# tinganchen/AlignQ

Measured on AMD Instinct MI355X. Metric: images/sec (train step, CDF+ADMM) ResNet-20 8-bit, higher is better.
Workload: dtype f32; 1 GPU; resnet20 CIFAR-shape 3x32x32, 8W/8A CDF+ADMM full train step (cdf_alignment_admm/resnet-20-cifar-10), batch 128/GPU, HIP-graph replay, batch-norm folded into the site kernels, channels-last tensors, all Conv2d_Q convolutions on alignq_conv*_nhwc (exact-product bf16 MFMA); global_batch=128, parallelism=dp1

## Files before the change

alignq_amd/csrc/conv_kernels.hip:

```cpp
#include <hip/hip_runtime.h>
#include <stdint.h>
#include <stdlib.h>

#include "../../include/alignq.h"
#include "site_internal.h"
#include "store_forms.h"
#include "wgrad_reduce_body.h"

namespace {

using namespace alignq_wgr;

typedef __bf16 bf16x8 __attribute__((ext_vector_type(8)));
typedef __bf16 bf16x4 __attribute__((ext_vector_type(4)));
typedef float f32x4 __attribute__((ext_vector_type(4)));
typedef short s16x4 __attribute__((ext_vector_type(4)));

#ifdef ALIGNQ_STAMPS
__device__ unsigned long long g_conv_stamps[64];
__device__ unsigned long long g_conv_blk[2][4096];
#define STAMP(on, i)                                                          \
  do {                                                                        \
    if ((on) && threadIdx.x == 0) g_conv_stamps[i] = wall_clock64();          \
  } while (0)
#define BSTAMP(which)                                                                          \
  do {                                                                                         \
    if (threadIdx.x == 0 && blockIdx.x < 4096) g_conv_blk[which][blockIdx.x] = wall_clock64(); \
  } while (0)
#else
#define STAMP(on, i) do { } while (0)
#define BSTAMP(which) do { } while (0)
#endif

__device__ __forceinline__ s16x4 tr_read(const __bf16* p) {
  return __builtin_amdgcn_ds_read_tr16_b64_v4i16((__attribute__((address_space(3))) s16x4*)(p));
}
__device__ __forceinline__ bf16x8 join8(s16x4 a, s16x4 b) {
  typedef short s16x8 __attribute__((ext_vector_type(8)));
  s16x8 v = {a[0], a[1], a[2], a[3], b[0], b[1], b[2], b[3]};
  return __builtin_bit_cast(bf16x8, v);
}


template <int xb>
__device__ __forceinline__ f32x4 fetch_act4(const float* __restrict__ x, int64_t off) {
  if constexpr (xb == 0) return *reinterpret_cast<const f32x4*>(x + off);
  if constexpr (xb == 2) {
    const s16x4 b = *reinterpret_cast<const s16x4*>(reinterpret_cast<const short*>(x) + off);
    return (f32x4){(float)b[0], (float)b[1], (float)b[2], (float)b[3]};
  }
  const char4 b = *reinterpret_cast<const char4*>(reinterpret_cast<const signed char*>(x) + off);
  return (f32x4){(float)b.x, (float)b.y, (float)b.z, (float)b.w};
}

struct BnLazy {
  const float* z;
  const float* ab;
  const float* save;
  const float* ktot;
  const float* part = nullptr;
  int n_tiles = 0, tile_f = 0;
  double inv_n = 1.0;
  float* dgamma = nullptr;
  float* dbeta = nullptr;
};

template <int C>
__device__ __forceinline__ void bn_totals_lds(const BnLazy& t, float* __restrict__ kt, bool publish) {
  static_assert(256 % C == 0, "thread -> (channel, group)");
  __shared__ double red[256][2];
  constexpr int G = 256 / C;
  const int tid = threadIdx.x;
  const int cp = C < t.tile_f ? C : t.tile_f;
  const int cyc = C / cp, cnt = t.n_tiles / cyc;
  const int c = tid % C, grp = tid / C;
  const int e = c % cp, t_first = c / cp;
  double s0 = 0, s1 = 0;
  constexpr int U = 16;
  for (int i0 = grp; i0 < cnt; i0 += G * U) {
    float2 v[U];
#pragma unroll
    for (int u = 0; u < U; u++) {
      const int i = i0 + u * G;
      const int ic = i < cnt ? i : cnt - 1;
      v[u] = *reinterpret_cast<const float2*>(t.part + ((int64_t)(ic * cyc + t_first) * cp + e) * 2);
    }
#pragma unroll
    for (int u = 0; u < U; u++) {
      if (i0 + u * G < cnt) { s0 += v[u].x; s1 += v[u].y; }
    }
  }
  red[tid][0] = s0;
  red[tid][1] = s1;
  __syncthreads();
  if (tid < C) {
    double t0 = 0, t1 = 0;
#pragma unroll
    for (int g = 0; g < G; g++) { t0 += red[g * C + tid][0]; t1 += red[g * C + tid][1]; }
    kt[tid] = (float)(t0 * t.inv_n);
    kt[C + tid] = (float)(t1 * t.inv_n);
    if (publish) {
      if (t.dbeta) t.dbeta[tid] = (float)t0;
      if (t.dgamma) t.dgamma[tid] = (float)t1;
    }
  }
  __syncthreads();
}

__device__ __forceinline__ float4 bn_lazy4(const float4& g, const float4& z, const float4& a, const float4& m, const float4& is,
                                           const float4& k0, const float4& k1) {
  float4 o;
  o.x = a.x * (g.x - k0.x - (z.x - m.x) * is.x * k1.x);
  o.y = a.y * (g.y - k0.y - (z.y - m.y) * is.y * k1.y);
  o.z = a.z * (g.z - k0.z - (z.z - m.z) * is.z * k1.z);
  o.w = a.w * (g.w - k0.w - (z.w - m.w) * is.w * k1.w);
  return o;
}

template <int C> constexpr int conv_cp() { return C == 16 ? 16 : (C == 32 ? 48 : C + 8); }
template <int C, int WD, int PT>
struct ConvLds {
  static constexpr int kBf16 = 3 * ((PT / WD) + 2) * (WD + 2) * conv_cp<C>();
};

template <int C, int WD, int PT, bool DGRAD, int XB = 0, bool IMG = false>
__device__ __forceinline__ void conv3x3_body(const float* __restrict__ x, const float* __restrict__ w,
                                             float* __restrict__ y, int H, int total_rows, float nlev, __bf16* lds,
                                             int block, const float* __restrict__ add,
                                             float* __restrict__ bn_part = nullptr, int n_wg = 0,
                                             BnLazy lazy = BnLazy{nullptr, nullptr, nullptr, nullptr}, float xlev = 1.0f) {
  static_assert(XB == 0 || !DGRAD, "the data gradient reads fp32 dy");
  constexpr int xb = XB;
  constexpr int TR = PT / WD;
  constexpr int NS = (9 * C + 31) / 32;
  constexpr int NCG = C / 16;
  constexpr int NPP = 4 / NCG;
  constexpr int NG = PT / 16;
  constexpr int LW = WD + 2;
  constexpr int CP = conv_cp<C>();
  constexpr int LROWS = TR + 2;
  constexpr int ARR = LROWS * LW * CP;
  static_assert(3 * ARR == ConvLds<C, WD, PT>::kBf16, "LDS size");
  __bf16* Xhi = lds;
  __bf16* Xmi = lds + ARR;
  __bf16* Xlo = lds + 2 * ARR;

  const int tid = threadIdx.x, lane = tid & 63, wv = tid >> 6;
  const int row0 = block * TR;
  const int img_lo = (row0 / H) * H, img_hi = img_lo + H;
  [[maybe_unused]] constexpr int SB = DGRAD ? 8 : 0;
  STAMP(block == 0, SB + 0);
  const int cog = wv % NCG, pp = wv / NCG;
  const int m = lane & 15, q = lane >> 4;
  bf16x8 ab[NS];
  {
    constexpr int C4 = C / 4;
    constexpr int N4 = LROWS * LW * C4;
    constexpr int NIT = (N4 + 255) / 256;
    float4 v[NIT];
#pragma unroll
    for (int it = 0; it < NIT; it++) {
      const int i = tid + 256 * it;
      const int c4 = i % C4, col = (i / C4) % LW, lr = i / (C4 * LW);
      const int grow = row0 + lr - 1;
      const bool ok = i < N4 && col >= 1 && col <= WD && grow >= img_lo && grow < img_hi && grow < total_rows;
      const int64_t off = ok ? ((int64_t)grow * WD + (col - 1)) * C + 4 * c4 : 0;
      const f32x4 ld = fetch_act4<XB>(x, off);
      v[it] = ok ? make_float4(ld[0], ld[1], ld[2], ld[3]) : make_float4(0.f, 0.f, 0.f, 0.f);
    }
    STAMP(block == 0, SB + 1);
    if (DGRAD && lazy.z) {
      float4 zz[NIT];
#pragma unroll
      for (int it = 0; it < NIT; it++) {
        const int i = tid + 256 * it;
        const int c4 = i % C4, col = (i / C4) % LW, lr = i / (C4 * LW);
        const int grow = row0 + lr - 1;
        const bool ok = i < N4 && col >= 1 && col <= WD && grow >= img_lo && grow < img_hi && grow < total_rows;
        zz[it] = *reinterpret_cast<const float4*>(lazy.z + (ok ? ((int64_t)grow * WD + (col - 1)) * C + 4 * c4 : 0));
      }
      const int c4t = tid % C4;
      const float4 a4 = *reinterpret_cast<const float4*>(lazy.ab + 4 * c4t);
      const float4 m4 = *reinterpret_cast<const float4*>(lazy.save + 4 * c4t);
      const float4 i4 = *reinterpret_cast<const float4*>(lazy.save + C + 4 * c4t);
      float4 k0, k1;
      if (lazy.part) {
        __shared__ __attribute__((aligned(16))) float kt[2 * C];
        bn_totals_lds<C>(lazy, kt, block == 0);
        k0 = *reinterpret_cast<const float4*>(kt + 4 * c4t);
        k1 = *reinterpret_cast<const float4*>(kt + C + 4 * c4t);
      } else {
        k0 = *reinterpret_cast<const float4*>(lazy.ktot + 4 * c4t);
        k1 = *reinterpret_cast<const float4*>(lazy.ktot + C + 4 * c4t);
      }
#pragma unroll
      for (int it = 0; it < NIT; it++) {
        const int i = tid + 256 * it;
        const int col = (i / C4) % LW, lr = i / (C4 * LW);
        const int grow = row0 + lr - 1;
        const bool ok = i < N4 && col >= 1 && col <= WD && grow >= img_lo && grow < img_hi && grow < total_rows;
        if (ok) v[it] = bn_lazy4(v[it], zz[it], a4, m4, i4, k0, k1);
      }
    }
#pragma unroll
    for (int it = 0; it < NIT; it++) {
      const int i = tid + 256 * it;
      if (i < N4) {
        const int c4 = i % C4, col = (i / C4) % LW, lr = i / (C4 * LW);
        bf16x4 h4, m4, l4;
        const float vv[4] = {v[it].x, v[it].y, v[it].z, v[it].w};
#pragma unroll
        for (int e = 0; e < 4; e++) {
          const __bf16 hi = (__bf16)vv[e];
          const float r1 = vv[e] - (float)hi;
          const __bf16 mi = (__bf16)r1;
          const float r2 = r1 - (float)mi;
          h4[e] = hi; m4[e] = mi; l4[e] = (__bf16)r2;
        }
        const int o = (lr * LW + col) * CP + 4 * c4;
        *reinterpret_cast<bf16x4*>(Xhi + o) = h4;
        *reinterpret_cast<bf16x4*>(Xmi + o) = m4;
        *reinterpret_cast<bf16x4*>(Xlo + o) = l4;
      }
    }
    STAMP(block == 0, SB + 2);
    if constexpr (IMG) {
      const bf16x8* __restrict__ wi = reinterpret_cast<const bf16x8*>(w) + (cog * NS) * 64 + lane;
#pragma unroll
      for (int s = 0; s < NS; s++) ab[s] = wi[s * 64];
    } else {
#pragma unroll
      for (int s = 0; s < NS; s++) {
        const int k0 = 32 * s + 8 * q;
        const bool live = k0 / C < 9;
        const int tap = live ? k0 / C : 8, c0 = k0 % C;
        float wr[8];
        if (!DGRAD) {
          const float* p = w + ((int64_t)(cog * 16 + m) * 9 + tap) * C + c0;
          const float4 a4 = *reinterpret_cast<const float4*>(p), b4 = *reinterpret_cast<const float4*>(p + 4);
          wr[0] = a4.x; wr[1] = a4.y; wr[2] = a4.z; wr[3] = a4.w; wr[4] = b4.x; wr[5] = b4.y; wr[6] = b4.z; wr[7] = b4.w;
        } else {
#pragma unroll
          for (int j = 0; j < 8; j++) wr[j] = w[((int64_t)(c0 + j) * 9 + (8 - tap)) * C + cog * 16 + m];
        }
#pragma unroll
        for (int j = 0; j < 8; j++) ab[s][j] = (__bf16)rintf((live ? wr[j] : 0.f) * nlev);
      }
    }
    STAMP(block == 0, SB + 3);
  }
  __syncthreads();
  constexpr int GW = NG / NPP;
  static_assert(NG % NPP == 0, "every wave takes the same number of pixel groups");
  int bo[GW];
  f32x4 acc[GW];
#pragma unroll
  for (int gi = 0; gi < GW; gi++) {
    const int p = (pp + gi * NPP) * 16 + (lane & 15);
    bo[gi] = ((p / WD) * LW + (p % WD)) * CP;
    acc[gi] = (f32x4){0.f, 0.f, 0.f, 0.f};
  }
  constexpr int GB = (DGRAD && GW > 2) ? 2 : GW;
  static_assert(GW % GB == 0, "whole batches of groups");
#pragma unroll
  for (int g0 = 0; g0 < GW; g0 += GB) {
    bf16x8 bh[2][GB], bm[2][GB], bl[2][GB];
#pragma unroll
    for (int s = 0; s <= NS; s++) {
      if (s < NS) {
        const int k0 = 32 * s + 8 * q;
        const bool live = k0 / C < 9;
        const int tap = live ? k0 / C : 8, c0 = k0 % C;
        const int to = ((tap / 3) * LW + (tap % 3)) * CP + c0;
#pragma unroll
        for (int gi = 0; gi < GB; gi++) {
          const int o = bo[g0 + gi] + to;
          bh[s & 1][gi] = *reinterpret_cast<const bf16x8*>(Xhi + o);
          bm[s & 1][gi] = *reinterpret_cast<const bf16x8*>(Xmi + o);
          if (DGRAD || xb == 0) bl[s & 1][gi] = *reinterpret_cast<const bf16x8*>(Xlo + o);
          if ((9 * C) % 32 != 0 && !live) {
#pragma unroll
            for (int j = 0; j < 8; j++) { bh[s & 1][gi][j] = (__bf16)0.f; bm[s & 1][gi][j] = (__bf16)0.f; bl[s & 1][gi][j] = (__bf16)0.f; }
          }
        }
      }
      __builtin_amdgcn_sched_barrier(0);
      if (s > 0) {
        const int u = s - 1;
#pragma unroll
        for (int gi = 0; gi < GB; gi++) {
          f32x4 a = acc[g0 + gi];
          if (DGRAD || xb == 0) a = __builtin_amdgcn_mfma_f32_16x16x32_bf16(ab[u], bl[u & 1][gi], a, 0, 0, 0);
          a = __builtin_amdgcn_mfma_f32_16x16x32_bf16(ab[u], bm[u & 1][gi], a, 0, 0, 0);
          acc[g0 + gi] = __builtin_amdgcn_mfma_f32_16x16x32_bf16(ab[u], bh[u & 1][gi], a, 0, 0, 0);
        }
      }
    }
  }
  float bs[4] = {0.f, 0.f, 0.f, 0.f}, bq[4] = {0.f, 0.f, 0.f, 0.f};
#pragma unroll
  for (int gi = 0; gi < GW; gi++) {
    const int p = (pp + gi * NPP) * 16 + (lane & 15);
    const int r = p / WD, c = p % WD;
    const int grow = row0 + r;
    if (grow < total_rows) {
      const int64_t o = ((int64_t)grow * WD + c) * C + cog * 16 + 4 * q;
      const float den = (!DGRAD && xb != 0) ? nlev * xlev : nlev;
      float4 v = make_float4(acc[gi][0] / den, acc[gi][1] / den, acc[gi][2] / den, acc[gi][3] / den);
      if (add) {
        const float4 r = *reinterpret_cast<const float4*>(add + o);
        v.x += r.x; v.y += r.y; v.z += r.z; v.w += r.w;
      }
      alignq_store::st16<alignq_store::kConvOut>(y + o, v);
      bs[0] += v.x; bs[1] += v.y; bs[2] += v.z; bs[3] += v.w;
      bq[0] += v.x * v.x; bq[1] += v.y * v.y; bq[2] += v.z * v.z; bq[3] += v.w * v.w;
    }
  }
  STAMP(block == 0, SB + 4);
  if (!DGRAD && bn_part) {
    float* red = reinterpret_cast<float*>(lds);
#define ROW_SHR_ADD(V, CTRL) V += __builtin_bit_cast(float, __builtin_amdgcn_update_dpp(0, __builtin_bit_cast(int, V), CTRL, 0xf, 0xf, false))
#pragma unroll
    for (int e = 0; e < 4; e++) {
      ROW_SHR_ADD(bs[e], 0x111); ROW_SHR_ADD(bs[e], 0x112); ROW_SHR_ADD(bs[e], 0x114); ROW_SHR_ADD(bs[e], 0x118);
      ROW_SHR_ADD(bq[e], 0x111); ROW_SHR_ADD(bq[e], 0x112); ROW_SHR_ADD(bq[e], 0x114); ROW_SHR_ADD(bq[e], 0x118);
    }
#undef ROW_SHR_ADD
    __syncthreads();
    if ((lane & 15) == 15) {
#pragma unroll
      for (int e = 0; e < 4; e++) {
        red[(wv * 16 + 4 * q + e) * 2] = bs[e];
        red[(wv * 16 + 4 * q + e) * 2 + 1] = bq[e];
      }
    }
    __syncthreads();
    if (tid < C) {
      const int cg = tid / 16, cl = tid % 16;
      float s0 = 0.f, s1 = 0.f;
#pragma unroll
      for (int ppi = 0; ppi < NPP; ppi++) {
        const int w2 = ppi * NCG + cg;
        s0 += red[(w2 * 16 + cl) * 2];
// ... 390 lines not shown
      float4 out = make_float4(acc[0] / nlev, acc[1] / nlev, acc[2] / nlev, acc[3] / nlev);
      if (add) {
        const float4 a4 = *reinterpret_cast<const float4*>(add + o);
        out.x += a4.x; out.y += a4.y; out.z += a4.z; out.w += a4.w;
      }
      alignq_store::st16<alignq_store::kConvOut>(dx + o, out);
    }
  }
}

template <int CIN, int COUT, int WDI, int KS, int PT, bool WITH1>
struct DgradS2Lds {
  static constexpr int P = KS == 3 ? 1 : 0, TR = PT / WDI;
  static constexpr int kBf16 = 3 * (((TR / 2 + P) * (WDI / 2 + P) + 1) + (WITH1 ? (TR / 2) * (WDI / 2) : 0)) * (COUT + 8);
};

template <int CIN, int COUT, int WDI, int KS, int PT, bool IMG = false>
__global__ __launch_bounds__(256) void dgrad_s2_kernel(const float* __restrict__ dy, const float* __restrict__ w,
                                                       float* __restrict__ dx, int H, int total_rows, float nlev,
                                                       const float* __restrict__ add, BnLazy lazy) {
  __shared__ __attribute__((aligned(16))) __bf16 lds[DgradS2Lds<CIN, COUT, WDI, KS, PT, false>::kBf16];
  dgrad_s2_body<CIN, COUT, WDI, KS, PT, false, IMG>(dy, w, dx, H, total_rows, nlev, add, lazy, lds, blockIdx.x);
}

template <int CIN, int COUT, int WDI, int KS, int PT>
int launch_dgrad_s2(const float* dy, const float* w, float* dx, int B, int H, float nlev, const float* add, BnLazy lazy,
                    hipStream_t st, bool img = false) {
  constexpr int TR = PT / WDI;
  static_assert(TR % 2 == 0, "even number of input rows per tile");
  if (H % TR) return ALIGNQ_EUNSUPPORTED;
  const int total_rows = B * H;
  if (img)
    hipLaunchKernelGGL((dgrad_s2_kernel<CIN, COUT, WDI, KS, PT, true>), total_rows / TR, 256, 0, st, dy, w, dx, H, total_rows, nlev,
                       add, lazy);
  else
    hipLaunchKernelGGL((dgrad_s2_kernel<CIN, COUT, WDI, KS, PT>), total_rows / TR, 256, 0, st, dy, w, dx, H, total_rows, nlev,
                       add, lazy);
  hipError_t e = hipGetLastError();
  return e == hipSuccess ? 0 : (int)e;
}

constexpr int kStemPT = 128;
__device__ __forceinline__ void stem_stage(const float* __restrict__ x, int H, int row0, __bf16* Chi, __bf16* Cmi, __bf16* Clo) {
  const int tid = threadIdx.x;
  const int pix = tid >> 1, half = tid & 1;
  const int r = pix / 32, c = pix % 32;
  const int grow = row0 + r;
  const int ih = grow % H;
  float v[16];
#pragma unroll
  for (int j = 0; j < 16; j++) {
    const int k = 16 * half + j;
    const int tap = k / 3, ci = k % 3;
    const int ky = tap / 3, kx = tap % 3;
    const int yy = ih + ky - 1, xx = c + kx - 1;
    const bool ok = k < 27 && yy >= 0 && yy < H && xx >= 0 && xx < 32;
    v[j] = x[ok ? ((int64_t)(grow + ky - 1) * 32 + xx) * 3 + ci : 0];
    if (!ok) v[j] = 0.f;
  }
  bf16x8 h[2], m[2], l[2];
#pragma unroll
  for (int j = 0; j < 16; j++) {
    const __bf16 hi = (__bf16)v[j];
    const float r1 = v[j] - (float)hi;
    const __bf16 mi = (__bf16)r1;
    h[j >> 3][j & 7] = hi; m[j >> 3][j & 7] = mi; l[j >> 3][j & 7] = (__bf16)(r1 - (float)mi);
  }
  const int o = pix * 32 + 16 * half;
  *reinterpret_cast<bf16x8*>(Chi + o) = h[0]; *reinterpret_cast<bf16x8*>(Chi + o + 8) = h[1];
  *reinterpret_cast<bf16x8*>(Cmi + o) = m[0]; *reinterpret_cast<bf16x8*>(Cmi + o + 8) = m[1];
  *reinterpret_cast<bf16x8*>(Clo + o) = l[0]; *reinterpret_cast<bf16x8*>(Clo + o + 8) = l[1];
}

__global__ __launch_bounds__(256) void stem_fwd_kernel(const float* __restrict__ x, const float* __restrict__ w,
                                                       float* __restrict__ y, int H, int total_rows, float nlev,
                                                       float* __restrict__ bn_part) {
  __shared__ __attribute__((aligned(16))) __bf16 lds[3 * kStemPT * 32];
  __bf16* Chi = lds;
  __bf16* Cmi = lds + kStemPT * 32;
  __bf16* Clo = lds + 2 * kStemPT * 32;
  const int tid = threadIdx.x, lane = tid & 63, wv = tid >> 6;
  const int row0 = blockIdx.x * 4;
  stem_stage(x, H, row0, Chi, Cmi, Clo);
  const int m = lane & 15, q = lane >> 4;
  bf16x8 ab;
#pragma unroll
  for (int j = 0; j < 8; j++) {
    const int k = 8 * q + j;
    ab[j] = (__bf16)rintf((k < 27 ? w[m * 27 + k] : 0.f) * nlev);
  }
  __syncthreads();
  float bs[4] = {0.f, 0.f, 0.f, 0.f}, bq[4] = {0.f, 0.f, 0.f, 0.f};
  for (int g = wv; g < kStemPT / 16; g += 4) {
    const int p = g * 16 + (lane & 15);
    const int o = p * 32 + 8 * q;
    f32x4 acc = {0.f, 0.f, 0.f, 0.f};
    acc = __builtin_amdgcn_mfma_f32_16x16x32_bf16(ab, *reinterpret_cast<const bf16x8*>(Clo + o), acc, 0, 0, 0);
    acc = __builtin_amdgcn_mfma_f32_16x16x32_bf16(ab, *reinterpret_cast<const bf16x8*>(Cmi + o), acc, 0, 0, 0);
    acc = __builtin_amdgcn_mfma_f32_16x16x32_bf16(ab, *reinterpret_cast<const bf16x8*>(Chi + o), acc, 0, 0, 0);
    const int grow = row0 + p / 32;
    if (grow < total_rows) {
      const float4 v = make_float4(acc[0] / nlev, acc[1] / nlev, acc[2] / nlev, acc[3] / nlev);
      alignq_store::st16<alignq_store::kConvOut>(y + ((int64_t)grow * 32 + p % 32) * 16 + 4 * q, v);
      bs[0] += v.x; bs[1] += v.y; bs[2] += v.z; bs[3] += v.w;
      bq[0] += v.x * v.x; bq[1] += v.y * v.y; bq[2] += v.z * v.z; bq[3] += v.w * v.w;
    }
  }
  if (bn_part) {
    float* red = reinterpret_cast<float*>(lds);
#define ROW_SHR_ADD(V, CTRL) V += __builtin_bit_cast(float, __builtin_amdgcn_update_dpp(0, __builtin_bit_cast(int, V), CTRL, 0xf, 0xf, false))
#pragma unroll
    for (int e = 0; e < 4; e++) {
      ROW_SHR_ADD(bs[e], 0x111); ROW_SHR_ADD(bs[e], 0x112); ROW_SHR_ADD(bs[e], 0x114); ROW_SHR_ADD(bs[e], 0x118);
      ROW_SHR_ADD(bq[e], 0x111); ROW_SHR_ADD(bq[e], 0x112); ROW_SHR_ADD(bq[e], 0x114); ROW_SHR_ADD(bq[e], 0x118);
    }
#undef ROW_SHR_ADD
    __syncthreads();
    if ((lane & 15) == 15) {
#pragma unroll
      for (int e = 0; e < 4; e++) {
        red[(wv * 16 + 4 * q + e) * 2] = bs[e];
        red[(wv * 16 + 4 * q + e) * 2 + 1] = bq[e];
      }
    }
    __syncthreads();
    if (tid < 16) {
      float s0 = 0.f, s1 = 0.f;
#pragma unroll
      for (int w2 = 0; w2 < 4; w2++) { s0 += red[(w2 * 16 + tid) * 2]; s1 += red[(w2 * 16 + tid) * 2 + 1]; }
      bn_part[((int64_t)tid * gridDim.x + blockIdx.x) * 2] = s0;
      bn_part[((int64_t)tid * gridDim.x + blockIdx.x) * 2 + 1] = s1;
    }
  }
}

__global__ __launch_bounds__(256) void stem_wgrad_kernel(const float* __restrict__ x, const float* __restrict__ dy,
                                                         float* __restrict__ slabs, int H, int n_tiles, BnLazy lazy) {
  __shared__ __attribute__((aligned(16))) __bf16 lds[3 * kStemPT * 32 + 3 * kStemPT * 16];
  __bf16* Ci[3] = {lds, lds + kStemPT * 32, lds + 2 * kStemPT * 32};
  __bf16* Di[3] = {lds + 3 * kStemPT * 32, lds + 3 * kStemPT * 32 + kStemPT * 16, lds + 3 * kStemPT * 32 + 2 * kStemPT * 16};
  const int tid = threadIdx.x, lane = tid & 63, wv = tid >> 6;
  const int g = lane >> 4, q = (lane & 15) >> 2, pcol = 4 * (lane & 3);
  f32x4 acc[2] = {{0.f, 0.f, 0.f, 0.f}, {0.f, 0.f, 0.f, 0.f}};
  __shared__ __attribute__((aligned(16))) float kt[32];
  if (lazy.z && lazy.part) bn_totals_lds<16>(lazy, kt, blockIdx.x == 0);
  for (int tile = blockIdx.x; tile < n_tiles; tile += gridDim.x) {
    const int row0 = tile * 4;
    f32x4 dvr[2], zvr[2];
#pragma unroll
    for (int it = 0; it < 2; it++) {
      const int i = tid + 256 * it;
      const int64_t off = ((int64_t)row0 * 32 + i / 4) * 16 + 4 * (tid % 4);
      dvr[it] = *reinterpret_cast<const f32x4*>(dy + off);
      zvr[it] = lazy.z ? *reinterpret_cast<const f32x4*>(lazy.z + off) : (f32x4){0.f, 0.f, 0.f, 0.f};
    }
    __syncthreads();
    stem_stage(x, H, row0, Ci[0], Ci[1], Ci[2]);
    {
      const int c4 = tid % 4;
      f32x4 la = {0, 0, 0, 0}, lm = la, li = la, lk0 = la, lk1 = la;
      if (lazy.z) {
        la = *reinterpret_cast<const f32x4*>(lazy.ab + 4 * c4);
        lm = *reinterpret_cast<const f32x4*>(lazy.save + 4 * c4);
        li = *reinterpret_cast<const f32x4*>(lazy.save + 16 + 4 * c4);
        const float* kp = lazy.part ? kt : lazy.ktot;
        lk0 = *reinterpret_cast<const f32x4*>(kp + 4 * c4);
        lk1 = *reinterpret_cast<const f32x4*>(kp + 16 + 4 * c4);
      }
#pragma unroll
      for (int it = 0; it < 2; it++) {
        const int i = tid + 256 * it;
        f32x4 dv = dvr[it];
        if (lazy.z) dv = la * (dv - lk0 - (zvr[it] - lm) * li * lk1);
        bf16x4 h4, m4, l4;
#pragma unroll
        for (int e = 0; e < 4; e++) {
          const __bf16 hi = (__bf16)dv[e];
          const float r1 = dv[e] - (float)hi;
          const __bf16 mi = (__bf16)r1;
          h4[e] = hi; m4[e] = mi; l4[e] = (__bf16)(r1 - (float)mi);
        }
        const int o = (i / 4) * 16 + 4 * c4;
        *reinterpret_cast<bf16x4*>(Di[0] + o) = h4;
        *reinterpret_cast<bf16x4*>(Di[1] + o) = m4;
        *reinterpret_cast<bf16x4*>(Di[2] + o) = l4;
      }
    }
    __syncthreads();
    {
      const int p0 = 32 * wv + 8 * g;
      bf16x8 a[3];
#pragma unroll
      for (int t = 0; t < 3; t++) {
        const __bf16* pa = Di[t] + (p0 + q) * 16 + pcol;
        a[t] = join8(tr_read(pa), tr_read(pa + 4 * 16));
      }
#pragma unroll
      for (int blk = 0; blk < 2; blk++) {
        bf16x8 b[3];
#pragma unroll
        for (int t = 0; t < 3; t++) {
          const __bf16* pb = Ci[t] + (p0 + q) * 32 + 16 * blk + pcol;
          b[t] = join8(tr_read(pb), tr_read(pb + 4 * 32));
        }
        f32x4 v = acc[blk];
        v = __builtin_amdgcn_mfma_f32_16x16x32_bf16(a[1], b[1], v, 0, 0, 0);
        v = __builtin_amdgcn_mfma_f32_16x16x32_bf16(a[0], b[2], v, 0, 0, 0);
        v = __builtin_amdgcn_mfma_f32_16x16x32_bf16(a[2], b[0], v, 0, 0, 0);
        v = __builtin_amdgcn_mfma_f32_16x16x32_bf16(a[0], b[1], v, 0, 0, 0);
        v = __builtin_amdgcn_mfma_f32_16x16x32_bf16(a[1], b[0], v, 0, 0, 0);
        v = __builtin_amdgcn_mfma_f32_16x16x32_bf16(a[0], b[0], v, 0, 0, 0);
        acc[blk] = v;
      }
    }
  }
  float* red = reinterpret_cast<float*>(lds);
  __syncthreads();
  if (wv > 0) {
#pragma unroll
    for (int blk = 0; blk < 2; blk++)
#pragma unroll
      for (int e = 0; e < 4; e++) red[(((wv - 1) * 2 + blk) * 4 + e) * 64 + lane] = acc[blk][e];
  }
  __syncthreads();
  if (wv == 0) {
    float* slab = slabs + (int64_t)blockIdx.x * (16 * 27);
#pragma unroll
    for (int blk = 0; blk < 2; blk++) {
#pragma unroll
      for (int e = 0; e < 4; e++) {
        float v = acc[blk][e];
#pragma unroll
        for (int w2 = 0; w2 < 3; w2++) v += red[((w2 * 2 + blk) * 4 + e) * 64 + lane];
        const int k = 16 * blk + (lane & 15), co = 4 * (lane >> 4) + e;
        if (k < 27) slab[co * 27 + k] = v;
      }
    }
  }
}

template <int CIN, int COUT, int WDI, int KS, int S, int PT>
int launch_gen(const float* x, const float* w, float* y, int B, int H, float nlev, float* bn_part, hipStream_t st,
               bool img = false) {
  constexpr int TR = ConvGen<CIN, COUT, WDI, KS, S, PT>::TR;
  if (H % TR) return ALIGNQ_EUNSUPPORTED;
  const int total_rows = B * H;
  if (img)
    hipLaunchKernelGGL((convgen_fwd_kernel<CIN, COUT, WDI, KS, S, PT, true>), total_rows / TR, 256, 0, st, x, w, y, H, total_rows,
                       nlev, bn_part);
  else
    hipLaunchKernelGGL((convgen_fwd_kernel<CIN, COUT, WDI, KS, S, PT>), total_rows / TR, 256, 0, st, x, w, y, H, total_rows,
                       nlev, bn_part);
  hipError_t e = hipGetLastError();
  return e == hipSuccess ? 0 : (int)e;
}

template <int C, int WD, int PT>
int launch(const float* x, const float* w, float* y, int B, int H, int dgrad, float nlev, const float* add, float* bn_part,
           hipStream_t st, int xb = 0, float xlev = 1.0f, bool img = false) {
  constexpr int TR = PT / WD;
  const int total_rows = B * H;
  if (H % TR) return ALIGNQ_EUNSUPPORTED;
  const int grid = total_rows / TR;
  if (img) {
    if (dgrad) hipLaunchKernelGGL((conv3x3_nhwc_kernel<C, WD, PT, true, 0, true>), grid, 256, 0, st, x, w, y, H, total_rows, nlev, add, nullptr, 1.0f);
    else if (xb == 2) hipLaunchKernelGGL((conv3x3_nhwc_kernel<C, WD, PT, false, 2, true>), grid, 256, 0, st, x, w, y, H, total_rows, nlev, add, bn_part, xlev);
    else if (xb == 1) hipLaunchKernelGGL((conv3x3_nhwc_kernel<C, WD, PT, false, 1, true>), grid, 256, 0, st, x, w, y, H, total_rows, nlev, add, bn_part, xlev);
    else hipLaunchKernelGGL((conv3x3_nhwc_kernel<C, WD, PT, false, 0, true>), grid, 256, 0, st, x, w, y, H, total_rows, nlev, add, bn_part, xlev);
  } else if (dgrad) hipLaunchKernelGGL((conv3x3_nhwc_kernel<C, WD, PT, true, 0>), grid, 256, 0, st, x, w, y, H, total_rows, nlev, add, nullptr, 1.0f);
  else if (xb == 2) hipLaunchKernelGGL((conv3x3_nhwc_kernel<C, WD, PT, false, 2>), grid, 256, 0, st, x, w, y, H, total_rows, nlev, add, bn_part, xlev);
  else if (xb == 1) hipLaunchKernelGGL((conv3x3_nhwc_kernel<C, WD, PT, false, 1>), grid, 256, 0, st, x, w, y, H, total_rows, nlev, add, bn_part, xlev);
  else hipLaunchKernelGGL((conv3x3_nhwc_kernel<C, WD, PT, false, 0>), grid, 256, 0, st, x, w, y, H, total_rows, nlev, add, bn_part, xlev);
  hipError_t e = hipGetLastError();
  return e == hipSuccess ? 0 : (int)e;
}

typedef float f32x16 __attribute__((ext_vector_type(16)));

template <int CIN, int COUT, int WDI, int KS, int S, int PT>
struct WgradGeo {
  static constexpr int WDO = WDI / S, TR = PT / WDO, NT = KS * KS;
  static constexpr int CB = (CIN < COUT ? CIN : COUT) >= 32 ? 32 : 16;
  static constexpr int XROWS = KS == 3 ? TR * S + (S == 1 ? 2 : 1) : TR;
  static constexpr int LW = KS == 3 ? WDI + 2 : WDO;
  static constexpr int XA = XROWS * LW * CB;
  static constexpr int DA = PT * CB;
  static constexpr int kRed = 3 * NT * 4 * 64 * 4;
  static constexpr int kBytes = (3 * (XA + DA) * 2) > kRed ? (3 * (XA + DA) * 2) : kRed;
  static constexpr int kFloats = kBytes / 4;
};
template <int C, int WD, int PT>
struct WgradLds : WgradGeo<C, C, WD, 3, 1, PT> {};

template <int CIN, int COUT, int WDI, int KS, int S, int PT, int XB = 0>
__device__ __forceinline__ void wgrad_body(const float* __restrict__ x, const float* __restrict__ dy,
                                           float* __restrict__ slabs, int H, int n_tiles, float* lds_f, int bx, int gx,
                                           int by, BnLazy lazy = BnLazy{nullptr, nullptr, nullptr, nullptr}, float xlev = 1.0f) {
  constexpr int xb = XB;
  using G = WgradGeo<CIN, COUT, WDI, KS, S, PT>;
  constexpr int WDO = G::WDO, TR = G::TR, NT = G::NT, CB = G::CB, LW = G::LW, XA = G::XA, DA = G::DA, XROWS = G::XROWS;
  constexpr int NBLK = CIN / CB;
  constexpr int NSTEP = PT / 32;
  static_assert(WDO % 8 == 0 && PT % 32 == 0, "a lane group's 8 pixels lie in one output row");
  __bf16* lds = reinterpret_cast<__bf16*>(lds_f);
  __bf16* Xi[3] = {lds, lds + XA, lds + 2 * XA};
  __bf16* Di[3] = {lds + 3 * XA, lds + 3 * XA + DA, lds + 3 * XA + 2 * DA};
  const int tid = threadIdx.x, lane = tid & 63, wv = tid >> 6;
  const int bi = by / NBLK, bj = by % NBLK;
  const int cob = CB == 32 ? (wv >> 1) : 0, cib = CB == 32 ? (wv & 1) : 0;
  const int g = lane >> 4, q = (lane & 15) >> 2, pcol = 4 * (lane & 3);

  [[maybe_unused]] const bool st_on = bx == 0 && by == 0;
  STAMP(st_on, 16);
  f32x4 acc[NT];
#pragma unroll
  for (int t = 0; t < NT; t++) acc[t] = (f32x4){0.f, 0.f, 0.f, 0.f};

  constexpr int C4 = CB / 4;
  constexpr int N4 = XROWS * LW * C4;
  constexpr int M4 = PT * C4;
  constexpr int NIX = (N4 + 255) / 256, NID = (M4 + 255) / 256;
  f32x4 rx[NIX], rd[NID], rz[NID];
  const int per = (n_tiles + gx - 1) / gx;
  const int t_begin = bx * per, t_end = (t_begin + per < n_tiles) ? t_begin + per : n_tiles;
  int nxt = t_begin;
  if (nxt < t_end) {
    const int row0_ = nxt * TR;
    const int img_lo_ = (row0_ / H) * (H * S), img_hi_ = img_lo_ + H * S;
#pragma unroll
    for (int it = 0; it < NIX; it++) {
      const int i = tid + 256 * it;
      const int c4 = i % C4, col = (i / C4) % LW, lr = i / (C4 * LW);
      const int grow = KS == 3 ? row0_ * S - 1 + lr : (row0_ + lr) * S;
      const int gcol = KS == 3 ? col - 1 : col * S;
      const bool ok = i < N4 && gcol >= 0 && gcol < WDI && grow >= img_lo_ && grow < img_hi_;
      const int64_t off = ok ? ((int64_t)grow * WDI + gcol) * CIN + bj * CB + 4 * c4 : 0;
      rx[it] = fetch_act4<XB>(x, off);
      if (!ok) rx[it] = (f32x4){0.f, 0.f, 0.f, 0.f};
    }
#pragma unroll
    for (int it = 0; it < NID; it++) {
      const int i = tid + 256 * it;
      const int64_t off = i < M4 ? ((int64_t)row0_ * WDO + i / C4) * COUT + bi * CB + 4 * (i % C4) : 0;
      rd[it] = *reinterpret_cast<const f32x4*>(dy + off);
      if (lazy.z) rz[it] = *reinterpret_cast<const f32x4*>(lazy.z + off);
    }
  }
  f32x4 la = {0, 0, 0, 0}, lm = la, li = la, lk0 = la, lk1 = la;
  if (lazy.z) {
    const int cq = bi * CB + 4 * (tid % C4);
    la = *reinterpret_cast<const f32x4*>(lazy.ab + cq);
    lm = *reinterpret_cast<const f32x4*>(lazy.save + cq);
    li = *reinterpret_cast<const f32x4*>(lazy.save + COUT + cq);
    if (lazy.part) {
      __shared__ __attribute__((aligned(16))) float kt[2 * COUT];
      bn_totals_lds<COUT>(lazy, kt, false);
      lk0 = *reinterpret_cast<const f32x4*>(kt + cq);
      lk1 = *reinterpret_cast<const f32x4*>(kt + COUT + cq);
    } else {
      lk0 = *reinterpret_cast<const f32x4*>(lazy.ktot + cq);
      lk1 = *reinterpret_cast<const f32x4*>(lazy.ktot + COUT + cq);
    }
  }
  STAMP(st_on, 17);
  for (int tile = t_begin; tile < t_end; tile++) {
    __syncthreads();
#pragma unroll
    for (int it = 0; it < NIX; it++) {
      const int i = tid + 256 * it;
      if (i < N4) {
        const int c4 = i % C4, col = (i / C4) % LW, lr = i / (C4 * LW);
        bf16x4 h4, m4, l4;
#pragma unroll
        for (int e = 0; e < 4; e++) {
          const float v = rx[it][e];
          const __bf16 hi = (__bf16)v;
          const float r1 = v - (float)hi;
          const __bf16 mi = (__bf16)r1;
          h4[e] = hi; m4[e] = mi; l4[e] = (__bf16)(r1 - (float)mi);
        }
        const int o = (lr * LW + col) * CB + 4 * c4;
        *reinterpret_cast<bf16x4*>(Xi[0] + o) = h4;
        *reinterpret_cast<bf16x4*>(Xi[1] + o) = m4;
        *reinterpret_cast<bf16x4*>(Xi[2] + o) = l4;
      }
    }
#pragma unroll
    for (int it = 0; it < NID; it++) {
      const int i = tid + 256 * it;
      if (i < M4) {
        bf16x4 h4, m4, l4;
        f32x4 dv = rd[it];
        if (lazy.z) dv = la * (dv - lk0 - (rz[it] - lm) * li * lk1);
#pragma unroll
        for (int e = 0; e < 4; e++) {
          const float v = dv[e];
          const __bf16 hi = (__bf16)v;
          const float r1 = v - (float)hi;
          const __bf16 mi = (__bf16)r1;
          h4[e] = hi; m4[e] = mi; l4[e] = (__bf16)(r1 - (float)mi);
        }
        const int o = (i / C4) * CB + 4 * (i % C4);
        *reinterpret_cast<bf16x4*>(Di[0] + o) = h4;
        *reinterpret_cast<bf16x4*>(Di[1] + o) = m4;
        *reinterpret_cast<bf16x4*>(Di[2] + o) = l4;
      }
    }
    __syncthreads();
    STAMP(st_on && tile - t_begin < 16, 18 + 2 * (tile - t_begin));
    nxt = tile + 1;
    if (nxt < t_end) {
      const int row0_ = nxt * TR;
      const int img_lo_ = (row0_ / H) * (H * S), img_hi_ = img_lo_ + H * S;
#pragma unroll
      for (int it = 0; it < NIX; it++) {
        const int i = tid + 256 * it;
        const int c4 = i % C4, col = (i / C4) % LW, lr = i / (C4 * LW);
        const int grow = KS == 3 ? row0_ * S - 1 + lr : (row0_ + lr) * S;
        const int gcol = KS == 3 ? col - 1 : col * S;
        const bool ok = i < N4 && gcol >= 0 && gcol < WDI && grow >= img_lo_ && grow < img_hi_;
        const int64_t off = ok ? ((int64_t)grow * WDI + gcol) * CIN + bj * CB + 4 * c4 : 0;
        rx[it] = fetch_act4<XB>(x, off);
        if (!ok) rx[it] = (f32x4){0.f, 0.f, 0.f, 0.f};
      }
#pragma unroll
      for (int it = 0; it < NID; it++) {
        const int i = tid + 256 * it;
        const int64_t off = i < M4 ? ((int64_t)row0_ * WDO + i / C4) * COUT + bi * CB + 4 * (i % C4) : 0;
        rd[it] = *reinterpret_cast<const f32x4*>(dy + off);
        if (lazy.z) rz[it] = *reinterpret_cast<const f32x4*>(lazy.z + off);
      }
    }
    for (int s = (CB == 16 ? wv : 0); s < NSTEP; s += (CB == 16 ? 4 : 1)) {
      const int p0 = 32 * s + 8 * g;
      const int r = p0 / WDO, c0 = p0 % WDO;
      bf16x8 a[3];
#pragma unroll
      for (int t = 0; t < 3; t++) {
        const __bf16* pa = Di[t] + (p0 + q) * CB + cob * 16 + pcol;
        a[t] = join8(tr_read(pa), tr_read(pa + 4 * CB));
      }
#pragma unroll
      for (int tap = 0; tap < NT; tap++) {
        const int ky = tap / KS, kx = tap % KS;
        bf16x8 b[3];
#pragma unroll
        for (int t = 0; t < 3; t++) {
          const __bf16* pb = Xi[t] + (KS == 3 ? ((r * S + ky) * LW + ((c0 + q) * S + kx)) : (r * LW + c0 + q)) * CB +
                             cib * 16 + pcol;
          b[t] = join8(tr_read(pb), tr_read(pb + 4 * (KS == 3 ? S : 1) * CB));
        }
        f32x4 v = acc[tap];
        v = __builtin_amdgcn_mfma_f32_16x16x32_bf16(a[1], b[1], v, 0, 0, 0);
        if (xb == 0) v = __builtin_amdgcn_mfma_f32_16x16x32_bf16(a[0], b[2], v, 0, 0, 0);
        v = __builtin_amdgcn_mfma_f32_16x16x32_bf16(a[2], b[0], v, 0, 0, 0);
        v = __builtin_amdgcn_mfma_f32_16x16x32_bf16(a[0], b[1], v, 0, 0, 0);
        v = __builtin_amdgcn_mfma_f32_16x16x32_bf16(a[1], b[0], v, 0, 0, 0);
        v = __builtin_amdgcn_mfma_f32_16x16x32_bf16(a[0], b[0], v, 0, 0, 0);
        acc[tap] = v;
      }
    }
    STAMP(st_on && tile - t_begin < 16, 19 + 2 * (tile - t_begin));
  }
  STAMP(st_on, 50);
  float* slab = slabs + (int64_t)bx * (NT * CIN * COUT);
  if (xb != 0) {
    const float inv = 1.0f / xlev;
#pragma unroll
    for (int t = 0; t < NT; t++) acc[t] = acc[t] * inv;
  }
  if (CB == 16) {
    float* red = lds_f;
    __syncthreads();
    if (wv > 0) {
#pragma unroll
      for (int t = 0; t < NT; t++)
#pragma unroll
        for (int e = 0; e < 4; e++) red[(((wv - 1) * NT + t) * 4 + e) * 64 + lane] = acc[t][e];
    }
    __syncthreads();
    if (wv == 0) {
#pragma unroll
      for (int t = 0; t < NT; t++) {
#pragma unroll
        for (int e = 0; e < 4; e++) {
          float v = acc[t][e];
#pragma unroll
          for (int w2 = 0; w2 < 3; w2++) v += red[((w2 * NT + t) * 4 + e) * 64 + lane];
          alignq_store::st4<alignq_store::kConvWgradSlab, true>(&slab[((int64_t)(bi * CB + 4 * (lane >> 4) + e) * NT + t) * CIN + bj * CB + (lane & 15)], v);
        }
      }
    }
  } else {
#pragma unroll
    for (int t = 0; t < NT; t++)
#pragma unroll
      for (int e = 0; e < 4; e++)
        alignq_store::st4<alignq_store::kConvWgradSlab, true>(&slab[((int64_t)(bi * CB + cob * 16 + 4 * (lane >> 4) + e) * NT + t) * CIN + bj * CB + cib * 16 + (lane & 15)], acc[t][e]);
  }
  STAMP(st_on, 51);
}

template <int C, int WD, int PT, int XB = 0>
__device__ __forceinline__ void wgrad3x3_body(const float* __restrict__ x, const float* __restrict__ dy,
                                              float* __restrict__ slabs, int H, int n_tiles, float* lds_f, int bx, int gx,
                                              int by, BnLazy lazy = BnLazy{nullptr, nullptr, nullptr, nullptr}, float xlev = 1.0f) {
  wgrad_body<C, C, WD, 3, 1, PT, XB>(x, dy, slabs, H, n_tiles, lds_f, bx, gx, by, lazy, xlev);
}

template <int CIN, int COUT, int WDI, int KS, int S, int PT>
__global__ __launch_bounds__(256) void wgradgen_kernel(const float* __restrict__ x, const float* __restrict__ dy,
                                                       float* __restrict__ slabs, int H, int n_tiles, BnLazy lazy) {
  __shared__ __attribute__((aligned(16))) float lds[WgradGeo<CIN, COUT, WDI, KS, S, PT>::kFloats];
  wgrad_body<CIN, COUT, WDI, KS, S, PT>(x, dy, slabs, H, n_tiles, lds, blockIdx.x, gridDim.x, blockIdx.y, lazy);
}

template <int C, int WD, int PT, int XB>
__global__ __launch_bounds__(256) void wgrad3x3_nhwc_kernel(const float* __restrict__ x, const float* __restrict__ dy,
                                                            float* __restrict__ slabs, int H, int n_tiles, float xlev) {
  __shared__ __attribute__((aligned(16))) float lds[WgradLds<C, WD, PT>::kFloats];
  wgrad3x3_body<C, WD, PT, XB>(x, dy, slabs, H, n_tiles, lds, blockIdx.x, gridDim.x, blockIdx.y,
                               BnLazy{nullptr, nullptr, nullptr, nullptr}, xlev);
}

template <int C, int WD, int PTD, int PTW, int XB, bool IMG = false>
__global__ __launch_bounds__(256) __attribute__((amdgpu_waves_per_eu(C == 16 ? 3 : 2, C == 16 ? 3 : 8)))
void conv3x3_bwd_kernel(const float* __restrict__ x, const float* __restrict__ dy,
                                                          const float* __restrict__ w, float* __restrict__ dx,
                                                          float* __restrict__ slabs, int H, int total_rows, float nlev,
                                                          int n_tiles_w, int splits, int nblk2,
                                                          const float* __restrict__ add, BnLazy lazy, float xlev, int dg_R,
                                                          RedFill fill, int n_dg) {
  constexpr int kBytesD = ConvLds<C, WD, PTD>::kBf16 * 2, kBytesW = WgradLds<C, WD, PTW>::kFloats * 4;
  static_assert(kBytesD >= 4096 || kBytesW >= 4096, "the filler role's 4 KB");
  __shared__ __attribute__((aligned(16))) unsigned char lds[kBytesD > kBytesW ? kBytesD : kBytesW];
  const int n_wg = splits * nblk2;
  BSTAMP(0);
  if ((int)blockIdx.x < n_wg) {
    wgrad3x3_body<C, WD, PTW, XB>(x, dy, slabs, H, n_tiles_w, reinterpret_cast<float*>(lds), blockIdx.x % splits, splits,
                                  blockIdx.x / splits, lazy, xlev);
  } else if ((int)blockIdx.x >= n_wg + n_dg) {
    const int fb = blockIdx.x - n_wg - n_dg;
    int it = 0;
    while (it + 1 < kFill && fb >= fill.blk0[it + 1]) it++;
    wgrad_reduce_body<256>(fill.slabs[it], fill.n_slabs[it], fill.n_elem[it], fill.dw[it], fb - fill.blk0[it],
                           reinterpret_cast<float*>(lds));
  } else {
    int m = blockIdx.x - n_wg;
    if (dg_R > 0) {
      const int i = (m / (8 * dg_R)) * 8 + (m & 7), r = (m >> 3) % dg_R;
      m = dg_R * i + r;
    }
    conv3x3_body<C, WD, PTD, true, 0, IMG>(dy, w, dx, H, total_rows, nlev, reinterpret_cast<__bf16*>(lds), m, add, nullptr, 0, lazy);
  }
  BSTAMP(1);
}

template <int CIN, int COUT, int WDI, int PTW3, int PTW1, int PTD, bool IMG = false>
__global__ __launch_bounds__(256) void transition_bwd_kernel(const float* __restrict__ x, const float* __restrict__ dy3,
                                                             const float* __restrict__ dy1, const float* __restrict__ w3,
                                                             const float* __restrict__ w1, float* __restrict__ dx,
                                                             float* __restrict__ slabs3, float* __restrict__ slabs1, int Ho,
                                                             int n_tiles3, int n_tiles1, int splits3, int splits1, int n_d,
                                                             float nlev, const float* __restrict__ add, BnLazy lazy3,
                                                             BnLazy lazy1, int dg_R) {
  using G3 = WgradGeo<CIN, COUT, WDI, 3, 2, PTW3>;
  using G1 = WgradGeo<CIN, COUT, WDI, 1, 2, PTW1>;
  constexpr int NBY = (COUT / G3::CB) * (CIN / G3::CB);
  static_assert(G3::CB == G1::CB, "same channel blocking");
  constexpr int kD = DgradS2Lds<CIN, COUT, WDI, 3, PTD, true>::kBf16 * 2;
  constexpr int kW = G3::kBytes > G1::kBytes ? G3::kBytes : G1::kBytes;
  __shared__ __attribute__((aligned(16))) unsigned char lds[kD > kW ? kD : kW];
  const int n_w3 = splits3 * NBY;
  const int b = blockIdx.x;
  if (b < n_d) {
    int m = b;
    if (dg_R > 0) {
      const int i = (m / (8 * dg_R)) * 8 + (m & 7), r = (m >> 3) % dg_R;
      m = dg_R * i + r;
    }
    dgrad_s2_body<CIN, COUT, WDI, 3, PTD, true, IMG>(dy3, w3, dx, 2 * Ho, 0x7fffffff, nlev, add, lazy3,
                                                     reinterpret_cast<__bf16*>(lds), m, dy1, w1, lazy1);
  } else if (b < n_d + n_w3) {
    const int c = b - n_d;
    wgrad_body<CIN, COUT, WDI, 3, 2, PTW3>(x, dy3, slabs3, Ho, n_tiles3, reinterpret_cast<float*>(lds), c % splits3, splits3,
                                           c / splits3, lazy3);
  } else {
    const int c = b - n_d - n_w3;
    wgrad_body<CIN, COUT, WDI, 1, 2, PTW1>(x, dy1, slabs1, Ho, n_tiles1, reinterpret_cast<float*>(lds), c % splits1, splits1,
                                           c / splits1, lazy1);
  }
}

__global__ __launch_bounds__(1024) void wgrad_reduce_kernel(const float* __restrict__ slabs, int n_slabs, int n_elem,
                                                            float* __restrict__ dw) {
  __shared__ __attribute__((aligned(16))) float part[4096];
  wgrad_reduce_body(slabs, n_slabs, n_elem, dw, blockIdx.x, part);
}

constexpr int kWgMulti = 32;
struct WgChunk {
  const float* slabs[kWgMulti];
  float* dw[kWgMulti];
  int n_slabs[kWgMulti];
  int n_elem[kWgMulti];
  int blk0[kWgMulti + 1];
};
__global__ __launch_bounds__(1024) void wgrad_reduce_multi_kernel(WgChunk c, int cnt) {
  __shared__ __attribute__((aligned(16))) float part[4096];
  int t = 0;
  while (t + 1 < cnt && (int)blockIdx.x >= c.blk0[t + 1]) t++;
  wgrad_reduce_body(c.slabs[t], c.n_slabs[t], c.n_elem[t], c.dw[t], (int)blockIdx.x - c.blk0[t], part);
}

template <int C, int WD, int PT>
int launch_wgrad(const float* x, const float* dy, float* dw, float* ws, int B, int H, int* n_slabs_out, hipStream_t st,
                 int xb = 0, float xlev = 1.0f) {
  constexpr int TR = PT / WD;
  if (H % TR) return ALIGNQ_EUNSUPPORTED;
  const int n_tiles = B * H / TR;
  constexpr int NB = (C >= 32 ? C / 32 : 1);
  int splits = 256 / (NB * NB);
  if (splits > n_tiles) splits = n_tiles;
  if (xb == 2) hipLaunchKernelGGL((wgrad3x3_nhwc_kernel<C, WD, PT, 2>), dim3(splits, NB * NB), 256, 0, st, x, dy, ws, H, n_tiles, xlev);
  else if (xb == 1) hipLaunchKernelGGL((wgrad3x3_nhwc_kernel<C, WD, PT, 1>), dim3(splits, NB * NB), 256, 0, st, x, dy, ws, H, n_tiles, xlev);
  else hipLaunchKernelGGL((wgrad3x3_nhwc_kernel<C, WD, PT, 0>), dim3(splits, NB * NB), 256, 0, st, x, dy, ws, H, n_tiles, xlev);
  hipError_t e = hipGetLastError();
  if (e != hipSuccess) return (int)e;
  if (n_slabs_out) { *n_slabs_out = splits; return 0; }
  const int n_elem = 9 * C * C;
  hipLaunchKernelGGL(wgrad_reduce_kernel, wgrad_reduce_blocks(splits, n_elem), 1024, 0, st, ws, splits, n_elem, dw);
  e = hipGetLastError();
  return e == hipSuccess ? 0 : (int)e;
}

template <int C, int WD, int PTD, int PTW>
int launch_bwd(const float* x, const float* dy, const float* w, float* dx, float* ws, int B, int H, float nlev,
               int* n_slabs_out, const float* add, BnLazy lazy, hipStream_t st, int xb, float xlev, const RedFill& fill,
               bool img) {
  constexpr int TRD = PTD / WD, TRW = PTW / WD;
  if (H % TRD || H % TRW) return ALIGNQ_EUNSUPPORTED;
  const int total_rows = B * H;
  const int n_tiles_w = total_rows / TRW;
  constexpr int NB = (C >= 32 ? C / 32 : 1);
  int splits = 256 / (NB * NB);
  if (splits > n_tiles_w) splits = n_tiles_w;
  const int n_d = total_rows / TRD;
  const int grid = splits * NB * NB + n_d + fill.blk0[kFill];
  const int per = (n_tiles_w + splits - 1) / splits;
  int dg_R = 0;
  if ((per * TRW) % TRD == 0 && (splits * NB * NB) % 8 == 0 && splits % 8 == 0) {
    const int R = per * TRW / TRD;
    if (R >= 1 && R * splits == n_d) dg_R = R;
  }
#define LBW(XBV, IM) hipLaunchKernelGGL((conv3x3_bwd_kernel<C, WD, PTD, PTW, XBV, IM>), grid, 256, 0, st, x, dy, w, dx, ws, H, total_rows, nlev, n_tiles_w, splits, NB * NB, add, lazy, xlev, dg_R, fill, n_d)
  if (img) {
    if (xb == 2) LBW(2, true); else if (xb == 1) LBW(1, true); else LBW(0, true);
  } else if (xb == 2) LBW(2, false); else if (xb == 1) LBW(1, false); else LBW(0, false);
#undef LBW
  hipError_t e = hipGetLastError();
  if (e != hipSuccess) return (int)e;
  *n_slabs_out = splits;
  return 0;
}

template <int CIN, int COUT, int WDI, int KS, int S, int PT>
int launch_wgradgen(const float* x, const float* dy, float* dw, float* ws, int B, int H, int* n_slabs_out, BnLazy lazy,
                    hipStream_t st) {
  using G = WgradGeo<CIN, COUT, WDI, KS, S, PT>;
  if (H % G::TR) return ALIGNQ_EUNSUPPORTED;
  const int n_tiles = B * H / G::TR;
  constexpr int NBY = (COUT / G::CB) * (CIN / G::CB);
  int splits = 256 / NBY;
  if (splits > n_tiles) splits = n_tiles;
  hipLaunchKernelGGL((wgradgen_kernel<CIN, COUT, WDI, KS, S, PT>), dim3(splits, NBY), 256, 0, st, x, dy, ws, H, n_tiles, lazy);
  hipError_t e = hipGetLastError();
  if (e != hipSuccess) return (int)e;
  if (n_slabs_out) { *n_slabs_out = splits; return 0; }
  const int n_elem = G::NT * CIN * COUT;
  hipLaunchKernelGGL(wgrad_reduce_kernel, wgrad_reduce_blocks(splits, n_elem), 1024, 0, st, ws, splits, n_elem, dw);
  e = hipGetLastError();
  return e == hipSuccess ? 0 : (int)e;
}

template <int CIN, int COUT, int WDI, int PT3, int PT1>
int launch_transition_fwd(const float* x, const float* w3, const float* w1, float* y3, float* y1, int B, int H, float nlev,
                          float* part3, float* part1, hipStream_t st, bool img) {
  constexpr int TR3 = ConvGen<CIN, COUT, WDI, 3, 2, PT3>::TR, TR1 = ConvGen<CIN, COUT, WDI, 1, 2, PT1>::TR;
  if (H % TR3 || H % TR1) return ALIGNQ_EUNSUPPORTED;
  const int total_rows = B * H, n3 = total_rows / TR3, n1 = total_rows / TR1;
  if (img)
    hipLaunchKernelGGL((transition_fwd_kernel<CIN, COUT, WDI, PT3, PT1, true>), n3 + n1, 256, 0, st, x, w3, w1, y3, y1, H,
                       total_rows, nlev, part3, part1, n3);
  else
    hipLaunchKernelGGL((transition_fwd_kernel<CIN, COUT, WDI, PT3, PT1>), n3 + n1, 256, 0, st, x, w3, w1, y3, y1, H, total_rows,
                       nlev, part3, part1, n3);
  hipError_t e = hipGetLastError();
  return e == hipSuccess ? 0 : (int)e;
}

template <int CIN, int COUT, int WDI, int PTW3, int PTW1, int PTD>
int launch_transition_bwd(const float* x, const float* dy3, const float* dy1, const float* w3, const float* w1, float* dx,
                          float* ws3, float* ws1, int B, int Ho, float nlev, int* ns3, int* ns1, const float* add,
                          BnLazy lazy3, BnLazy lazy1, hipStream_t st, bool img) {
  using G3 = WgradGeo<CIN, COUT, WDI, 3, 2, PTW3>;
  using G1 = WgradGeo<CIN, COUT, WDI, 1, 2, PTW1>;
  constexpr int TRD = PTD / WDI;
  if (Ho % G3::TR || Ho % G1::TR || (2 * Ho) % TRD) return ALIGNQ_EUNSUPPORTED;
  const int n_tiles3 = B * Ho / G3::TR, n_tiles1 = B * Ho / G1::TR;
  constexpr int NBY = (COUT / G3::CB) * (CIN / G3::CB);
  int splits3 = 256 / NBY, splits1 = 256 / NBY;
  if (splits3 > n_tiles3) splits3 = n_tiles3;
  if (splits1 > n_tiles1) splits1 = n_tiles1;
  const int n_d = B * 2 * Ho / TRD;
  int dg_R = 0;
  {
    const int per3 = (n_tiles3 + splits3 - 1) / splits3, per1 = (n_tiles1 + splits1 - 1) / splits1;
    const int rows3 = per3 * G3::TR, rows1 = per1 * G1::TR;
    if (rows3 == rows1 && splits3 == splits1 && splits3 % 8 == 0 && n_d % 8 == 0 && (2 * rows3) % TRD == 0) {
      const int R = 2 * rows3 / TRD;
      if (R >= 1 && R * splits3 == n_d) dg_R = R;
    }
  }
  if (img)
    hipLaunchKernelGGL((transition_bwd_kernel<CIN, COUT, WDI, PTW3, PTW1, PTD, true>), (splits3 + splits1) * NBY + n_d, 256, 0, st,
                       x, dy3, dy1, w3, w1, dx, ws3, ws1, Ho, n_tiles3, n_tiles1, splits3, splits1, n_d, nlev, add, lazy3, lazy1,
                       dg_R);
  else
    hipLaunchKernelGGL((transition_bwd_kernel<CIN, COUT, WDI, PTW3, PTW1, PTD>), (splits3 + splits1) * NBY + n_d, 256, 0, st, x,
                       dy3, dy1, w3, w1, dx, ws3, ws1, Ho, n_tiles3, n_tiles1, splits3, splits1, n_d, nlev, add, lazy3, lazy1,
                       dg_R);
  hipError_t e = hipGetLastError();
  if (e != hipSuccess) return (int)e;
  *ns3 = splits3;
  *ns1 = splits1;
  return 0;
}

}

static int lazy_parts(BnLazy& lazy, const float* dx_part, float* dgamma, float* dbeta, int B, int C, int HW) {
  if (!lazy.z || lazy.ktot || !dx_part) return 0;
  const int64_t F = (int64_t)C * HW;
  const int tf = alignq_site::bwd_tile_features(B, F);
  if (F % tf || (C > tf && C % tf) || (C < tf && tf % C)) return ALIGNQ_EUNSUPPORTED;
  lazy.part = dx_part; lazy.n_tiles = (int)(F / tf); lazy.tile_f = tf; lazy.inv_n = 1.0 / ((double)B * HW);
  lazy.dgamma = dgamma; lazy.dbeta = dbeta;
  return 0;
}

extern "C" {

int alignq_conv3x3_bn_parts(int B, int H, int W, int C) {
  const int pt = (C == 16 && W == 32) ? 256 : (C == 32 && W == 16) ? 128 : (C == 64 && W == 8) ? 32 : 0;
  if (!pt || B < 1 || H < 1 || H % (pt / W)) return 0;
  return B * H / (pt / W);
}

static int act_bins_ok(const void* x_bins, int x_bin_bytes, int a_bit) {
  if (!x_bins) return 1;
  return (x_bin_bytes == 1 || x_bin_bytes == 2) && a_bit >= 1 && a_bit <= 16 && !(reinterpret_cast<uintptr_t>(x_bins) & 15);
}
// ... 390 lines not shown
```

Measured before the change: 141,300 images/sec.

## Share row transpose-reads across kx taps in wgrad and skip unused low split

```diff
diff --git a/alignq_amd/csrc/conv_kernels.hip b/alignq_amd/csrc/conv_kernels.hip
--- a/alignq_amd/csrc/conv_kernels.hip
+++ b/alignq_amd/csrc/conv_kernels.hip
@@ -39,6 +39,18 @@
   typedef short s16x8 __attribute__((ext_vector_type(8)));
   s16x8 v = {a[0], a[1], a[2], a[3], b[0], b[1], b[2], b[3]};
   return __builtin_bit_cast(bf16x8, v);
+}
+__device__ __forceinline__ void row_frags(s16x4 r0, s16x4 r1, s16x4 r2, bf16x8& f0, bf16x8& f1, bf16x8& f2) {
+  typedef unsigned u32x2 __attribute__((ext_vector_type(2)));
+  typedef unsigned u32x4 __attribute__((ext_vector_type(4)));
+  const u32x2 a = __builtin_bit_cast(u32x2, r0), b = __builtin_bit_cast(u32x2, r1), c = __builtin_bit_cast(u32x2, r2);
+  const u32x4 v0 = {a[0], a[1], b[0], b[1]};
+  const u32x4 v1 = {__builtin_amdgcn_alignbit(a[1], a[0], 16), __builtin_amdgcn_alignbit(b[0], a[1], 16),
+                    __builtin_amdgcn_alignbit(b[1], b[0], 16), __builtin_amdgcn_alignbit(c[0], b[1], 16)};
+  const u32x4 v2 = {a[1], b[0], b[1], c[0]};
+  f0 = __builtin_bit_cast(bf16x8, v0);
+  f1 = __builtin_bit_cast(bf16x8, v1);
+  f2 = __builtin_bit_cast(bf16x8, v2);
 }
 
 
@@ -1035,6 +1047,14 @@
   constexpr int NBLK = CIN / CB;
   constexpr int NSTEP = PT / 32;
   static_assert(WDO % 8 == 0 && PT % 32 == 0, "a lane group's 8 pixels lie in one output row");
+#ifdef ALIGNQ_WGRAD_TAP_READS
+  constexpr bool kRowReads = false;
+  constexpr int NXT = 3;
+#else
+  constexpr bool kRowReads = KS == 3 && S == 1 && !(CIN == 32 && xb == 0);
+  constexpr int NXT = xb != 0 ? 2 : 3;
+#endif
+  static_assert(!kRowReads || DA >= 2 * CB, "the row run's over-read stays inside the LDS allocation");
   __bf16* lds = reinterpret_cast<__bf16*>(lds_f);
   __bf16* Xi[3] = {lds, lds + XA, lds + 2 * XA};
   __bf16* Di[3] = {lds + 3 * XA, lds + 3 * XA + DA, lds + 3 * XA + 2 * DA};
@@ -1103,19 +1123,21 @@
       const int i = tid + 256 * it;
       if (i < N4) {
         const int c4 = i % C4, col = (i / C4) % LW, lr = i / (C4 * LW);
-        bf16x4 h4, m4, l4;
+        bf16x4 h4, m4;
+        [[maybe_unused]] bf16x4 l4;
 #pragma unroll
         for (int e = 0; e < 4; e++) {
           const float v = rx[it][e];
           const __bf16 hi = (__bf16)v;
           const float r1 = v - (float)hi;
           const __bf16 mi = (__bf16)r1;
-          h4[e] = hi; m4[e] = mi; l4[e] = (__bf16)(r1 - (float)mi);
+          h4[e] = hi; m4[e] = mi;
+          if constexpr (NXT == 3) l4[e] = (__bf16)(r1 - (float)mi);
         }
         const int o = (lr * LW + col) * CB + 4 * c4;
         *reinterpret_cast<bf16x4*>(Xi[0] + o) = h4;
         *reinterpret_cast<bf16x4*>(Xi[1] + o) = m4;
-        *reinterpret_cast<bf16x4*>(Xi[2] + o) = l4;
+        if constexpr (NXT == 3) *reinterpret_cast<bf16x4*>(Xi[2] + o) = l4;
       }
     }
 #pragma unroll
@@ -1173,24 +1195,52 @@
         const __bf16* pa = Di[t] + (p0 + q) * CB + cob * 16 + pcol;
         a[t] = join8(tr_read(pa), tr_read(pa + 4 * CB));
       }
-#pragma unroll
-      for (int tap = 0; tap < NT; tap++) {
-        const int ky = tap / KS, kx = tap % KS;
-        bf16x8 b[3];
-#pragma unroll
-        for (int t = 0; t < 3; t++) {
-          const __bf16* pb = Xi[t] + (KS == 3 ? ((r * S + ky) * LW + ((c0 + q) * S + kx)) : (r * LW + c0 + q)) * CB +
-                             cib * 16 + pcol;
-          b[t] = join8(tr_read(pb), tr_read(pb + 4 * (KS == 3 ? S : 1) * CB));
+      if constexpr (kRowReads) {
+#pragma unroll
+        for (int ky = 0; ky < 3; ky++) {
+          bf16x8 b0[3], b1[3], b2[3];
+          const __bf16* pb = Xi[0] + ((r + ky) * LW + c0 + q) * CB + cib * 16 + pcol;
+          row_frags(tr_read(pb + XA), tr_read(pb + XA + 4 * CB), tr_read(pb + XA + 8 * CB), b1[0], b1[1], b1[2]);
+#pragma unroll
+          for (int kx = 0; kx < 3; kx++)
+            acc[3 * ky + kx] = __builtin_amdgcn_mfma_f32_16x16x32_bf16(a[1], b1[kx], acc[3 * ky + kx], 0, 0, 0);
+          if constexpr (NXT == 3) {
+            row_frags(tr_read(pb + 2 * XA), tr_read(pb + 2 * XA + 4 * CB), tr_read(pb + 2 * XA + 8 * CB), b2[0], b2[1], b2[2]);
+#pragma unroll
+            for (int kx = 0; kx < 3; kx++)
+              acc[3 * ky + kx] = __builtin_amdgcn_mfma_f32_16x16x32_bf16(a[0], b2[kx], acc[3 * ky + kx], 0, 0, 0);
+          }
+          row_frags(tr_read(pb), tr_read(pb + 4 * CB), tr_read(pb + 8 * CB), b0[0], b0[1], b0[2]);
+#pragma unroll
+          for (int kx = 0; kx < 3; kx++) {
+            f32x4 v = acc[3 * ky + kx];
+            v = __builtin_amdgcn_mfma_f32_16x16x32_bf16(a[2], b0[kx], v, 0, 0, 0);
+            v = __builtin_amdgcn_mfma_f32_16x16x32_bf16(a[0], b1[kx], v, 0, 0, 0);
+            v = __builtin_amdgcn_mfma_f32_16x16x32_bf16(a[1], b0[kx], v, 0, 0, 0);
+            v = __builtin_amdgcn_mfma_f32_16x16x32_bf16(a[0], b0[kx], v, 0, 0, 0);
+            acc[3 * ky + kx] = v;
+          }
         }
-        f32x4 v = acc[tap];
-        v = __builtin_amdgcn_mfma_f32_16x16x32_bf16(a[1], b[1], v, 0, 0, 0);
-        if (xb == 0) v = __builtin_amdgcn_mfma_f32_16x16x32_bf16(a[0], b[2], v, 0, 0, 0);
-        v = __builtin_amdgcn_mfma_f32_16x16x32_bf16(a[2], b[0], v, 0, 0, 0);
-        v = __builtin_amdgcn_mfma_f32_16x16x32_bf16(a[0], b[1], v, 0, 0, 0);
-        v = __builtin_amdgcn_mfma_f32_16x16x32_bf16(a[1], b[0], v, 0, 0, 0);
-        v = __builtin_amdgcn_mfma_f32_16x16x32_bf16(a[0], b[0], v, 0, 0, 0);
-        acc[tap] = v;
+      } else {
+#pragma unroll
+        for (int tap = 0; tap < NT; tap++) {
+          const int ky = tap / KS, kx = tap % KS;
+          bf16x8 b[3];
+#pragma unroll
+          for (int t = 0; t < 3; t++) {
+            const __bf16* pb = Xi[t] + (KS == 3 ? ((r * S + ky) * LW + ((c0 + q) * S + kx)) : (r * LW + c0 + q)) * CB +
+                               cib * 16 + pcol;
+            b[t] = join8(tr_read(pb), tr_read(pb + 4 * (KS == 3 ? S : 1) * CB));
+          }
+          f32x4 v = acc[tap];
+          v = __builtin_amdgcn_mfma_f32_16x16x32_bf16(a[1], b[1], v, 0, 0, 0);
+          if (xb == 0) v = __builtin_amdgcn_mfma_f32_16x16x32_bf16(a[0], b[2], v, 0, 0, 0);
+          v = __builtin_amdgcn_mfma_f32_16x16x32_bf16(a[2], b[0], v, 0, 0, 0);
+          v = __builtin_amdgcn_mfma_f32_16x16x32_bf16(a[0], b[1], v, 0, 0, 0);
+          v = __builtin_amdgcn_mfma_f32_16x16x32_bf16(a[1], b[0], v, 0, 0, 0);
+          v = __builtin_amdgcn_mfma_f32_16x16x32_bf16(a[0], b[0], v, 0, 0, 0);
+          acc[tap] = v;
+        }
       }
     }
     STAMP(st_on && tile - t_begin < 16, 19 + 2 * (tile - t_begin));
```

Result: no change. 140,700 images/sec (-0.5%).
